# facebookresearch/co-tracker

Hardware: NVIDIA H100
Metric: tracked points*frames/sec at N=6400, T=16, 512^2 (higher is better)
Workload: dtype transformer + corr_mlp.fc2 + input_transform: bf16x3; correlation einsum: fp16x2; corr_mlp.fc1: bf16x3; fp32 accumulate, fp32 softmax/LayerNorm/GELU

## Files before the change

### cotracker_b200/csrc/common.cuh

```cuda
#pragma once
#include <cuda.h>
#include <cuda_bf16.h>
#include <cuda_fp16.h>
#include <cuda_runtime.h>
#include <stdint.h>

#include <atomic>

namespace ct3 {

struct DeviceOnce { std::atomic<uint64_t> done[2] = {}; };
template <typename F>
inline cudaError_t once_per_device(DeviceOnce& flag, F&& f) {
  int dev = 0;
  cudaError_t e = cudaGetDevice(&dev);
  if (e != cudaSuccess) return e;
  if (dev < 0 || dev >= 128) return f();
  const uint64_t bit = 1ull << (dev & 63);
  if (flag.done[dev >> 6].load(std::memory_order_acquire) & bit) return cudaSuccess;
  e = f();
  if (e == cudaSuccess) flag.done[dev >> 6].fetch_or(bit, std::memory_order_release);
  return e;
}

// ... 178 lines not shown
  uint64_t p;
  asm volatile("createpolicy.fractional.L2::evict_last.b64 %0, 1.0;" : "=l"(p));
  return p;
}
__device__ __forceinline__ void tma_load_4d_hint(void* smem_dst, const CUtensorMap* m, int c0, int c1, int c2, int c3,
                                                 uint64_t* bar, uint64_t policy) {
  asm volatile(
      "cp.async.bulk.tensor.4d.shared::cluster.global.mbarrier::complete_tx::bytes.L2::cache_hint [%0], [%1, {%3, %4, %5, %6}], [%2], %7;"
      ::"r"(smem_u32(smem_dst)), "l"(reinterpret_cast<uint64_t>(m)), "r"(smem_u32(bar)), "r"(c0), "r"(c1), "r"(c2),
      "r"(c3), "l"(policy)
      : "memory");
}
__device__ __forceinline__ void tma_load_3d(void* smem_dst, const CUtensorMap* m, int c0, int c1, int c2, uint64_t* bar) {
  asm volatile(
      "cp.async.bulk.tensor.3d.shared::cluster.global.mbarrier::complete_tx::bytes [%0], [%1, {%3, %4, %5}], [%2];"
      ::"r"(smem_u32(smem_dst)), "l"(reinterpret_cast<uint64_t>(m)), "r"(smem_u32(bar)), "r"(c0), "r"(c1), "r"(c2)
      : "memory");
}
__device__ __forceinline__ void tma_store_3d(const CUtensorMap* m, int c0, int c1, int c2, const void* smem_src) {
  asm volatile("cp.async.bulk.tensor.3d.global.shared::cta.bulk_group [%0, {%2, %3, %4}], [%1];"
               ::"l"(reinterpret_cast<uint64_t>(m)), "r"(smem_u32(smem_src)), "r"(c0), "r"(c1), "r"(c2)
               : "memory");
}

__device__ __forceinline__ void bulk_store_s2g(void* gdst, const void* ssrc, uint32_t bytes) {
  asm volatile("cp.async.bulk.global.shared::cta.bulk_group [%0], [%1], %2;" ::"l"(gdst), "r"(smem_u32(ssrc)), "r"(bytes)
               : "memory");
}
__device__ __forceinline__ void bulk_store_s2g_hint(void* gdst, const void* ssrc, uint32_t bytes, uint64_t policy) {
  asm volatile("cp.async.bulk.global.shared::cta.bulk_group.L2::cache_hint [%0], [%1], %2, %3;" ::"l"(gdst),
               "r"(smem_u32(ssrc)), "r"(bytes), "l"(policy)
               : "memory");
}
__device__ __forceinline__ void bulk_commit() { asm volatile("cp.async.bulk.commit_group;" ::: "memory"); }
__device__ __forceinline__ void bulk_wait_read0() { asm volatile("cp.async.bulk.wait_group.read 0;" ::: "memory"); }
__device__ __forceinline__ void bulk_wait0() { asm volatile("cp.async.bulk.wait_group 0;" ::: "memory"); }

__device__ __forceinline__ uint64_t gmma_desc_sw128(uint32_t smem_addr) {
  uint64_t d = 0;
  d |= (uint64_t)((smem_addr & 0x3FFFFu) >> 4);
  d |= (uint64_t)1 << 16;
  d |= (uint64_t)(1024 >> 4) << 32;
  d |= (uint64_t)1 << 62;
  return d;
}
__device__ __forceinline__ void wgmma_fence() { asm volatile("wgmma.fence.sync.aligned;" ::: "memory"); }
__device__ __forceinline__ void wgmma_commit() { asm volatile("wgmma.commit_group.sync.aligned;" ::: "memory"); }
template <int R>
__device__ __forceinline__ void wgmma_wait0(float (&d)[R]) {
  asm volatile("wgmma.wait_group.sync.aligned 0;" ::: "memory");
#pragma unroll
  for (int i = 0; i < R; ++i) asm volatile("" : "+f"(d[i])::"memory");
}

__device__ __forceinline__ void wgmma_m64n64_bf16(float (&d)[32], uint64_t da, uint64_t db, uint32_t scale_d) {
  asm volatile(
      "{\n\t.reg .pred p;\n\tsetp.ne.b32 p, %34, 0;\n\t"
      "wgmma.mma_async.sync.aligned.m64n64k16.f32.bf16.bf16 "
      "{%0, %1, %2, %3, %4, %5, %6, %7, %8, %9, %10, %11, %12, %13, %14, %15, %16, %17, %18, %19, %20, %21, %22, %23, %24, %25, %26, %27, %28, %29, %30, %31}, %32, %33, p, 1, 1, 0, 0;\n\t}"
      : "+f"(d[0]), "+f"(d[1]), "+f"(d[2]), "+f"(d[3]), "+f"(d[4]), "+f"(d[5]), "+f"(d[6]), "+f"(d[7]), "+f"(d[8]), "+f"(d[9]), "+f"(d[10]), "+f"(d[11]), "+f"(d[12]), "+f"(d[13]), "+f"(d[14]), "+f"(d[15]), "+f"(d[16]), "+f"(d[17]), "+f"(d[18]), "+f"(d[19]), "+f"(d[20]), "+f"(d[21]), "+f"(d[22]), "+f"(d[23]), "+f"(d[24]), "+f"(d[25]), "+f"(d[26]), "+f"(d[27]), "+f"(d[28]), "+f"(d[29]), "+f"(d[30]), "+f"(d[31])
      : "l"(da), "l"(db), "r"(scale_d));
}
__device__ __forceinline__ void wgmma_m64n128_bf16(float (&d)[64], uint64_t da, uint64_t db, uint32_t scale_d) {
  asm volatile(
      "{\n\t.reg .pred p;\n\tsetp.ne.b32 p, %66, 0;\n\t"
      "wgmma.mma_async.sync.aligned.m64n128k16.f32.bf16.bf16 "
      "{%0, %1, %2, %3, %4, %5, %6, %7, %8, %9, %10, %11, %12, %13, %14, %15, %16, %17, %18, %19, %20, %21, %22, %23, %24, %25, %26, %27, %28, %29, %30, %31, %32, %33, %34, %35, %36, %37, %38, %39, %40, %41, %42, %43, %44, %45, %46, %47, %48, %49, %50, %51, %52, %53, %54, %55, %56, %57, %58, %59, %60, %61, %62, %63}, %64, %65, p, 1, 1, 0, 0;\n\t}"
      : "+f"(d[0]), "+f"(d[1]), "+f"(d[2]), "+f"(d[3]), "+f"(d[4]), "+f"(d[5]), "+f"(d[6]), "+f"(d[7]), "+f"(d[8]), "+f"(d[9]), "+f"(d[10]), "+f"(d[11]), "+f"(d[12]), "+f"(d[13]), "+f"(d[14]), "+f"(d[15]), "+f"(d[16]), "+f"(d[17]), "+f"(d[18]), "+f"(d[19]), "+f"(d[20]), "+f"(d[21]), "+f"(d[22]), "+f"(d[23]), "+f"(d[24]), "+f"(d[25]), "+f"(d[26]), "+f"(d[27]), "+f"(d[28]), "+f"(d[29]), "+f"(d[30]), "+f"(d[31]), "+f"(d[32]), "+f"(d[33]), "+f"(d[34]), "+f"(d[35]), "+f"(d[36]), "+f"(d[37]), "+f"(d[38]), "+f"(d[39]), "+f"(d[40]), "+f"(d[41]), "+f"(d[42]), "+f"(d[43]), "+f"(d[44]), "+f"(d[45]), "+f"(d[46]), "+f"(d[47]), "+f"(d[48]), "+f"(d[49]), "+f"(d[50]), "+f"(d[51]), "+f"(d[52]), "+f"(d[53]), "+f"(d[54]), "+f"(d[55]), "+f"(d[56]), "+f"(d[57]), "+f"(d[58]), "+f"(d[59]), "+f"(d[60]), "+f"(d[61]), "+f"(d[62]), "+f"(d[63])
      : "l"(da), "l"(db), "r"(scale_d));
}
__device__ __forceinline__ void wgmma_m64n144_bf16(float (&d)[72], uint64_t da, uint64_t db, uint32_t scale_d) {
  asm volatile(
      "{\n\t.reg .pred p;\n\tsetp.ne.b32 p, %74, 0;\n\t"
      "wgmma.mma_async.sync.aligned.m64n144k16.f32.bf16.bf16 "
      "{%0, %1, %2, %3, %4, %5, %6, %7, %8, %9, %10, %11, %12, %13, %14, %15, %16, %17, %18, %19, %20, %21, %22, %23, %24, %25, %26, %27, %28, %29, %30, %31, %32, %33, %34, %35, %36, %37, %38, %39, %40, %41, %42, %43, %44, %45, %46, %47, %48, %49, %50, %51, %52, %53, %54, %55, %56, %57, %58, %59, %60, %61, %62, %63, %64, %65, %66, %67, %68, %69, %70, %71}, %72, %73, p, 1, 1, 0, 0;\n\t}"
      : "+f"(d[0]), "+f"(d[1]), "+f"(d[2]), "+f"(d[3]), "+f"(d[4]), "+f"(d[5]), "+f"(d[6]), "+f"(d[7]), "+f"(d[8]), "+f"(d[9]), "+f"(d[10]), "+f"(d[11]), "+f"(d[12]), "+f"(d[13]), "+f"(d[14]), "+f"(d[15]), "+f"(d[16]), "+f"(d[17]), "+f"(d[18]), "+f"(d[19]), "+f"(d[20]), "+f"(d[21]), "+f"(d[22]), "+f"(d[23]), "+f"(d[24]), "+f"(d[25]), "+f"(d[26]), "+f"(d[27]), "+f"(d[28]), "+f"(d[29]), "+f"(d[30]), "+f"(d[31]), "+f"(d[32]), "+f"(d[33]), "+f"(d[34]), "+f"(d[35]), "+f"(d[36]), "+f"(d[37]), "+f"(d[38]), "+f"(d[39]), "+f"(d[40]), "+f"(d[41]), "+f"(d[42]), "+f"(d[43]), "+f"(d[44]), "+f"(d[45]), "+f"(d[46]), "+f"(d[47]), "+f"(d[48]), "+f"(d[49]), "+f"(d[50]), "+f"(d[51]), "+f"(d[52]), "+f"(d[53]), "+f"(d[54]), "+f"(d[55]), "+f"(d[56]), "+f"(d[57]), "+f"(d[58]), "+f"(d[59]), "+f"(d[60]), "+f"(d[61]), "+f"(d[62]), "+f"(d[63]), "+f"(d[64]), "+f"(d[65]), "+f"(d[66]), "+f"(d[67]), "+f"(d[68]), "+f"(d[69]), "+f"(d[70]), "+f"(d[71])
      : "l"(da), "l"(db), "r"(scale_d));
}
__device__ __forceinline__ void wgmma_m64n64_f16(float (&d)[32], uint64_t da, uint64_t db, uint32_t scale_d) {
  asm volatile(
      "{\n\t.reg .pred p;\n\tsetp.ne.b32 p, %34, 0;\n\t"
      "wgmma.mma_async.sync.aligned.m64n64k16.f32.f16.f16 "
      "{%0, %1, %2, %3, %4, %5, %6, %7, %8, %9, %10, %11, %12, %13, %14, %15, %16, %17, %18, %19, %20, %21, %22, %23, %24, %25, %26, %27, %28, %29, %30, %31}, %32, %33, p, 1, 1, 0, 0;\n\t}"
      : "+f"(d[0]), "+f"(d[1]), "+f"(d[2]), "+f"(d[3]), "+f"(d[4]), "+f"(d[5]), "+f"(d[6]), "+f"(d[7]), "+f"(d[8]), "+f"(d[9]), "+f"(d[10]), "+f"(d[11]), "+f"(d[12]), "+f"(d[13]), "+f"(d[14]), "+f"(d[15]), "+f"(d[16]), "+f"(d[17]), "+f"(d[18]), "+f"(d[19]), "+f"(d[20]), "+f"(d[21]), "+f"(d[22]), "+f"(d[23]), "+f"(d[24]), "+f"(d[25]), "+f"(d[26]), "+f"(d[27]), "+f"(d[28]), "+f"(d[29]), "+f"(d[30]), "+f"(d[31])
      : "l"(da), "l"(db), "r"(scale_d));
}
__device__ __forceinline__ void wgmma_m64n128_f16(float (&d)[64], uint64_t da, uint64_t db, uint32_t scale_d) {
  asm volatile(
      "{\n\t.reg .pred p;\n\tsetp.ne.b32 p, %66, 0;\n\t"
      "wgmma.mma_async.sync.aligned.m64n128k16.f32.f16.f16 "
      "{%0, %1, %2, %3, %4, %5, %6, %7, %8, %9, %10, %11, %12, %13, %14, %15, %16, %17, %18, %19, %20, %21, %22, %23, %24, %25, %26, %27, %28, %29, %30, %31, %32, %33, %34, %35, %36, %37, %38, %39, %40, %41, %42, %43, %44, %45, %46, %47, %48, %49, %50, %51, %52, %53, %54, %55, %56, %57, %58, %59, %60, %61, %62, %63}, %64, %65, p, 1, 1, 0, 0;\n\t}"
      : "+f"(d[0]), "+f"(d[1]), "+f"(d[2]), "+f"(d[3]), "+f"(d[4]), "+f"(d[5]), "+f"(d[6]), "+f"(d[7]), "+f"(d[8]), "+f"(d[9]), "+f"(d[10]), "+f"(d[11]), "+f"(d[12]), "+f"(d[13]), "+f"(d[14]), "+f"(d[15]), "+f"(d[16]), "+f"(d[17]), "+f"(d[18]), "+f"(d[19]), "+f"(d[20]), "+f"(d[21]), "+f"(d[22]), "+f"(d[23]), "+f"(d[24]), "+f"(d[25]), "+f"(d[26]), "+f"(d[27]), "+f"(d[28]), "+f"(d[29]), "+f"(d[30]), "+f"(d[31]), "+f"(d[32]), "+f"(d[33]), "+f"(d[34]), "+f"(d[35]), "+f"(d[36]), "+f"(d[37]), "+f"(d[38]), "+f"(d[39]), "+f"(d[40]), "+f"(d[41]), "+f"(d[42]), "+f"(d[43]), "+f"(d[44]), "+f"(d[45]), "+f"(d[46]), "+f"(d[47]), "+f"(d[48]), "+f"(d[49]), "+f"(d[50]), "+f"(d[51]), "+f"(d[52]), "+f"(d[53]), "+f"(d[54]), "+f"(d[55]), "+f"(d[56]), "+f"(d[57]), "+f"(d[58]), "+f"(d[59]), "+f"(d[60]), "+f"(d[61]), "+f"(d[62]), "+f"(d[63])
      : "l"(da), "l"(db), "r"(scale_d));
}
__device__ __forceinline__ void wgmma_m64n144_f16(float (&d)[72], uint64_t da, uint64_t db, uint32_t scale_d) {
  asm volatile(
      "{\n\t.reg .pred p;\n\tsetp.ne.b32 p, %74, 0;\n\t"
      "wgmma.mma_async.sync.aligned.m64n144k16.f32.f16.f16 "
      "{%0, %1, %2, %3, %4, %5, %6, %7, %8, %9, %10, %11, %12, %13, %14, %15, %16, %17, %18, %19, %20, %21, %22, %23, %24, %25, %26, %27, %28, %29, %30, %31, %32, %33, %34, %35, %36, %37, %38, %39, %40, %41, %42, %43, %44, %45, %46, %47, %48, %49, %50, %51, %52, %53, %54, %55, %56, %57, %58, %59, %60, %61, %62, %63, %64, %65, %66, %67, %68, %69, %70, %71}, %72, %73, p, 1, 1, 0, 0;\n\t}"
      : "+f"(d[0]), "+f"(d[1]), "+f"(d[2]), "+f"(d[3]), "+f"(d[4]), "+f"(d[5]), "+f"(d[6]), "+f"(d[7]), "+f"(d[8]), "+f"(d[9]), "+f"(d[10]), "+f"(d[11]), "+f"(d[12]), "+f"(d[13]), "+f"(d[14]), "+f"(d[15]), "+f"(d[16]), "+f"(d[17]), "+f"(d[18]), "+f"(d[19]), "+f"(d[20]), "+f"(d[21]), "+f"(d[22]), "+f"(d[23]), "+f"(d[24]), "+f"(d[25]), "+f"(d[26]), "+f"(d[27]), "+f"(d[28]), "+f"(d[29]), "+f"(d[30]), "+f"(d[31]), "+f"(d[32]), "+f"(d[33]), "+f"(d[34]), "+f"(d[35]), "+f"(d[36]), "+f"(d[37]), "+f"(d[38]), "+f"(d[39]), "+f"(d[40]), "+f"(d[41]), "+f"(d[42]), "+f"(d[43]), "+f"(d[44]), "+f"(d[45]), "+f"(d[46]), "+f"(d[47]), "+f"(d[48]), "+f"(d[49]), "+f"(d[50]), "+f"(d[51]), "+f"(d[52]), "+f"(d[53]), "+f"(d[54]), "+f"(d[55]), "+f"(d[56]), "+f"(d[57]), "+f"(d[58]), "+f"(d[59]), "+f"(d[60]), "+f"(d[61]), "+f"(d[62]), "+f"(d[63]), "+f"(d[64]), "+f"(d[65]), "+f"(d[66]), "+f"(d[67]), "+f"(d[68]), "+f"(d[69]), "+f"(d[70]), "+f"(d[71])
      : "l"(da), "l"(db), "r"(scale_d));
}

__device__ __forceinline__ void wgmma_m64n48_bf16(float (&d)[24], uint64_t da, uint64_t db, uint32_t scale_d) {
  asm volatile(
      "{\n\t.reg .pred p;\n\tsetp.ne.b32 p, %26, 0;\n\t"
// ... 91 lines not shown
```

### cotracker_b200/csrc/gemm.cu

```cuda
#include "gemm.cuh"

namespace ct3 {
namespace {

constexpr int BM = 128, BN = 128, BK = 64;
constexpr int TILE_A = BM * BK * 2;
constexpr int TILE_B = BN * BK * 2;
constexpr int MMA_WARPS = 4;
constexpr int TMA_WARP = 4;
constexpr int EPI_WARP0 = 8;
constexpr int EPI_WARPS = 8;
constexpr int CW = 16;
constexpr int STG_WORDS = 32 * CW;
constexpr int MAX_STAGES = 4;
template <int NPROD>
struct Cfg {
  static constexpr int AP = NPROD >= 3 ? 2 : 1;
  static constexpr int BP = NPROD >= 2 ? 2 : 1;
  static constexpr int STAGE_BYTES = AP * TILE_A + BP * TILE_B;
  static constexpr int STAGES = NPROD >= 2 ? 2 : 4;
  static constexpr int OFF_B = AP * TILE_A;
};
constexpr int RING_BYTES = 2 * 65536;
static_assert(Cfg<1>::STAGES * Cfg<1>::STAGE_BYTES <= RING_BYTES && Cfg<2>::STAGES * Cfg<2>::STAGE_BYTES <= RING_BYTES &&
              Cfg<3>::STAGES * Cfg<3>::STAGE_BYTES <= RING_BYTES, "ring size");
constexpr int ACC_LD = BN + 4;
constexpr int OFF_ACC = RING_BYTES;
constexpr int OFF_STG = OFF_ACC + BM * ACC_LD * 4;
constexpr int OFF_BAR = OFF_STG + EPI_WARPS * STG_WORDS * 4;
constexpr int SMEM_BYTES = OFF_BAR + 256  + 1024 ;
static_assert(SMEM_BYTES <= 232448, "shared memory budget");
constexpr int THREADS = (EPI_WARP0 + EPI_WARPS) * 32;
constexpr int REG_TMA = 40, REG_MMA = 216, REG_EPI = 65536 / THREADS;
static_assert(128 * (REG_TMA + REG_MMA + 2 * REG_EPI) <= 65536, "register budget");

__device__ __forceinline__ float apply_act(float x, int act) {
  if (act == 1) return gelu_erf(x);
  if (act == 2) return gelu_tanh(x);
  return x;
}

__device__ __forceinline__ int stg_idx(int row, int word) { return row * CW + ((word + (row >> 1)) & (CW - 1)); }

__device__ __forceinline__ void epilogue_chunk(const GemmEpilogue& e, int M, int N, int row0, int col0, int lane,
                                               float (&v)[CW], uint32_t* stg) {
  const int row = row0 + lane;
  if (e.bias) {
    const float4* b4 = reinterpret_cast<const float4*>(e.bias + col0);
#pragma unroll
    for (int i = 0; i < CW / 4; ++i) {
      float4 b = __ldg(b4 + i);
      v[4 * i + 0] += b.x; v[4 * i + 1] += b.y; v[4 * i + 2] += b.z; v[4 * i + 3] += b.w;
    }
  }
  if (e.row_bias && row < M) {
    const float4* b4 = reinterpret_cast<const float4*>(e.row_bias + (int64_t)(row % e.row_mod) * N + col0);
#pragma unroll
    for (int i = 0; i < CW / 4; ++i) {
      float4 b = __ldg(b4 + i);
      v[4 * i + 0] += b.x; v[4 * i + 1] += b.y; v[4 * i + 2] += b.z; v[4 * i + 3] += b.w;
    }
  }
  if (e.act != 0) {
#pragma unroll
    for (int i = 0; i < CW; ++i) v[i] = apply_act(v[i], e.act);
  }
  const int rsub = lane >> 2, q = lane & 3;
  if (e.out_f32) {
#pragma unroll
    for (int c = 0; c < CW; ++c) stg[stg_idx(lane, c)] = __float_as_uint(v[c]);
    __syncwarp();
    float* base = e.out_f32 + (int64_t)(row0 + rsub) * e.ld_f32 + col0 + 4 * q;
    const int64_t rstep = 8 * e.ld_f32;
    float4 x[4];
#pragma unroll
    for (int k = 0; k < 4; ++k) {
      const int r = 8 * k + rsub;
      x[k] = make_float4(__uint_as_float(stg[stg_idx(r, 4 * q + 0)]), __uint_as_float(stg[stg_idx(r, 4 * q + 1)]),
                         __uint_as_float(stg[stg_idx(r, 4 * q + 2)]), __uint_as_float(stg[stg_idx(r, 4 * q + 3)]));
    }
    if (e.residual) {
      float4 r4[4];
#pragma unroll
      for (int k = 0; k < 4; ++k)
        r4[k] = (row0 + 8 * k + rsub < M) ? *reinterpret_cast<const float4*>(base + k * rstep) : make_float4(0.f, 0.f, 0.f, 0.f);
#pragma unroll
      for (int k = 0; k < 4; ++k) { x[k].x += r4[k].x; x[k].y += r4[k].y; x[k].z += r4[k].z; x[k].w += r4[k].w; }
    }
#pragma unroll
    for (int k = 0; k < 4; ++k)
      if (row0 + 8 * k + rsub < M) *reinterpret_cast<float4*>(base + k * rstep) = x[k];
    __syncwarp();
  }
  if (e.out_split) {
#pragma unroll
    for (int i = 0; i < CW / 2; ++i) {
      uint32_t hi, lo;
      split2(v[2 * i], v[2 * i + 1], hi, lo);
      stg[stg_idx(lane, i)] = hi;
      stg[stg_idx(lane, CW / 2 + i)] = lo;
    }
    __syncwarp();
    uint32_t off16_lane = 0xffffffffu;
    if (row < M) {
      const int orow = row / e.row_group;
      off16_lane = (uint32_t)(((long long)orow * e.ld_split + (long long)(row % e.row_group) * N + col0) >> 3);
    }
    uint4* plane = reinterpret_cast<uint4*>(e.out_split + (q >= 2 ? e.lo_off : 0)) + (q & 1);
#pragma unroll
    for (int k = 0; k < 4; ++k) {
      const int r = 8 * k + rsub;
      const uint32_t o16 = __shfl_sync(0xffffffffu, off16_lane, r);
      const uint4 w4 = make_uint4(stg[stg_idx(r, 4 * q + 0)], stg[stg_idx(r, 4 * q + 1)], stg[stg_idx(r, 4 * q + 2)],
                                  stg[stg_idx(r, 4 * q + 3)]);
      if (o16 != 0xffffffffu) plane[o16] = w4;
    }
    __syncwarp();
  }
}

template <int NPROD>
__global__ void __launch_bounds__(THREADS, 1)
gemm_split3_tc_kernel(const __grid_constant__ CUtensorMap tmX, const __grid_constant__ CUtensorMap tmW, int M,
                      int N, int Kpad, int fp16, GemmEpilogue epi) {
  using C = Cfg<NPROD>;
  constexpr int STAGES = C::STAGES, STAGE_BYTES = C::STAGE_BYTES;
  extern __shared__ __align__(1024) uint8_t smem_raw[];
  uint8_t* smem = smem_align1024(smem_raw);
  uint64_t* full_bar = reinterpret_cast<uint64_t*>(smem + OFF_BAR);
  uint64_t* empty_bar = full_bar + MAX_STAGES;
  uint64_t* tfull_bar = empty_bar + MAX_STAGES;
  uint64_t* tempty_bar = tfull_bar + 1;
  float* acc_tile = reinterpret_cast<float*>(smem + OFF_ACC);

  const int warp = threadIdx.x >> 5, lane = threadIdx.x & 31;

  if (threadIdx.x == 0) {
    tma_prefetch_desc(&tmX);
    tma_prefetch_desc(&tmW);
    for (int i = 0; i < STAGES; ++i) {
      mbar_init(&full_bar[i], 1);
      mbar_init(&empty_bar[i], MMA_WARPS);
    }
    mbar_init(tfull_bar, MMA_WARPS);
    mbar_init(tempty_bar, EPI_WARPS * 32);
    fence_barrier_init();
  }
  __syncthreads();

  const int num_mt = (M + BM - 1) / BM;
  const int num_nt = N / BN;
  const int num_tiles = num_mt * num_nt;
  const int num_kb = Kpad / BK;

  if (warp >= MMA_WARPS && warp < EPI_WARP0) {
    setmaxnreg_dec<REG_TMA>();
    if (warp == TMA_WARP && elect_one()) {
      int stage = 0;
      uint32_t phase = 0;
      for (int tile = blockIdx.x; tile < num_tiles; tile += gridDim.x) {
        const int mt = tile / num_nt, nt = tile % num_nt;
        for (int kb = 0; kb < num_kb; ++kb) {
          mbar_wait(&empty_bar[stage], phase ^ 1u);
          mbar_arrive_expect_tx(&full_bar[stage], STAGE_BYTES);
          uint8_t* s = smem + stage * STAGE_BYTES;
          tma_load_2d(s, &tmX, kb * BK, mt * BM, &full_bar[stage]);
          if (C::AP == 2) tma_load_2d(s + TILE_A, &tmX, Kpad + kb * BK, mt * BM, &full_bar[stage]);
          tma_load_2d(s + C::OFF_B, &tmW, kb * BK, nt * BN, &full_bar[stage]);
          if (C::BP == 2) tma_load_2d(s + C::OFF_B + TILE_B, &tmW, Kpad + kb * BK, nt * BN, &full_bar[stage]);
          if (++stage == STAGES) { stage = 0; phase ^= 1u; }
        }
      }
    }
  } else if (warp < MMA_WARPS) {
    setmaxnreg_inc<REG_MMA>();
    int stage = 0;
    uint32_t phase = 0, acc_phase = 0;
    for (int tile = blockIdx.x; tile < num_tiles; tile += gridDim.x) {
      float d0[BN / 2], d1[BN / 2];
      for (int kb = 0; kb < num_kb; ++kb) {
        mbar_wait(&full_bar[stage], phase);
        wgmma_fence();
        const uint32_t sa = smem_u32(smem + stage * STAGE_BYTES);
        if (fp16) mma_kblock<NPROD, BN, true>(d0, d1, sa, TILE_A, C::OFF_B, TILE_B, kb == 0);
        else mma_kblock<NPROD, BN, false>(d0, d1, sa, TILE_A, C::OFF_B, TILE_B, kb == 0);
        wgmma_commit();
        wgmma_wait0(d0);
        wgmma_wait0(d1);
        __syncwarp();
        if (lane == 0) mbar_arrive(&empty_bar[stage]);
        if (++stage == STAGES) { stage = 0; phase ^= 1u; }
      }
      mbar_wait(tempty_bar, acc_phase ^ 1u);
      acc_store<BN>(d0, acc_tile, ACC_LD);
      acc_store<BN>(d1, acc_tile + 64 * ACC_LD, ACC_LD);
      __syncwarp();
      if (lane == 0) mbar_arrive(tfull_bar);
      acc_phase ^= 1u;
    }
  } else {
    const int e = warp - EPI_WARP0;
    const int quarter = e & 3;
    constexpr int CH = BN / CW / (EPI_WARPS / 4);
    const int chunk0 = (e >> 2) * CH;
    uint32_t acc_phase = 0;
    for (int tile = blockIdx.x; tile < num_tiles; tile += gridDim.x) {
      const int mt = tile / num_nt, nt = tile % num_nt;
      mbar_wait(tfull_bar, acc_phase);
      const int row0 = mt * BM + quarter * 32;
      uint32_t* stg = reinterpret_cast<uint32_t*>(smem + OFF_STG) + e * STG_WORDS;
      const float* arow = acc_tile + (quarter * 32 + lane) * ACC_LD;
#pragma unroll 1
      for (int chunk = chunk0; chunk < chunk0 + CH; ++chunk) {
        float v[CW];
        acc_row_ld<CW>(arow + chunk * CW, v);
        epilogue_chunk(epi, M, N, row0, nt * BN + chunk * CW, lane, v, stg);
      }
      mbar_arrive(tempty_bar);
      acc_phase ^= 1u;
    }
  }
}

namespace qa {
constexpr int BNQ = 144;
constexpr int TILE_BQ = BNQ * BK * 2;
constexpr int STAGE = 2 * TILE_A + 2 * TILE_BQ;
constexpr int NSTAGE = 2;
constexpr int QACC_LD = BNQ + 4;
constexpr int QOFF_ACC = NSTAGE * STAGE;
constexpr int OFF_BARQ = QOFF_ACC + BM * QACC_LD * 4;
constexpr int SMEM = OFF_BARQ + 256 + 1024;
constexpr int EPIW = 4;
constexpr int QEPI_WARP0 = 8;
constexpr int NTHREADS = 12 * 32;
constexpr int REG_PRODUCER = 40, REG_COMPUTE = 232;
static_assert(128 * (REG_PRODUCER + 2 * REG_COMPUTE) <= NTHREADS * 168, "register budget");
static_assert(SMEM <= 232448, "shared memory budget");
}

__global__ void __launch_bounds__(qa::NTHREADS, 1)
gemm_qkv_time_attn_kernel(const __grid_constant__ CUtensorMap tmX, const __grid_constant__ CUtensorMap tmW, int M,
                          int Kpad, int T, int R, float scale_log2e, GemmEpilogue epi) {
  using namespace qa;
  extern __shared__ __align__(1024) uint8_t smem_raw[];
  uint8_t* smem = smem_align1024(smem_raw);
  uint64_t* full_bar = reinterpret_cast<uint64_t*>(smem + OFF_BARQ);
  uint64_t* empty_bar = full_bar + NSTAGE;
  uint64_t* tfull_bar = empty_bar + NSTAGE;
  uint64_t* tempty_bar = tfull_bar + 1;
  float* acc = reinterpret_cast<float*>(smem + QOFF_ACC);

  const int warp = threadIdx.x >> 5, lane = threadIdx.x & 31;
  if (threadIdx.x == 0) {
    tma_prefetch_desc(&tmX);
    tma_prefetch_desc(&tmW);
    for (int i = 0; i < NSTAGE; ++i) {
      mbar_init(&full_bar[i], 1);
      mbar_init(&empty_bar[i], MMA_WARPS);
    }
    mbar_init(tfull_bar, MMA_WARPS);
    mbar_init(tempty_bar, EPIW * 32);
    fence_barrier_init();
  }
  __syncthreads();

  const int num_mt = (M + R - 1) / R;
  const int num_tiles = num_mt * kHeads;
  const int num_kb = Kpad / BK;

  if (warp >= MMA_WARPS && warp < QEPI_WARP0) {
    setmaxnreg_dec<REG_PRODUCER>();
    if (warp == TMA_WARP && elect_one()) {
      int stage = 0;
      uint32_t phase = 0;
      for (int tile = blockIdx.x; tile < num_tiles; tile += gridDim.x) {
        const int mt = tile / kHeads, h = tile % kHeads;
        for (int kb = 0; kb < num_kb; ++kb) {
          mbar_wait(&empty_bar[stage], phase ^ 1u);
          mbar_arrive_expect_tx(&full_bar[stage], STAGE);
          uint8_t* s = smem + stage * STAGE;
          tma_load_2d(s, &tmX, kb * BK, mt * R, &full_bar[stage]);
          tma_load_2d(s + TILE_A, &tmX, Kpad + kb * BK, mt * R, &full_bar[stage]);
          tma_load_2d(s + 2 * TILE_A, &tmW, kb * BK, h * BNQ, &full_bar[stage]);
          tma_load_2d(s + 2 * TILE_A + TILE_BQ, &tmW, Kpad + kb * BK, h * BNQ, &full_bar[stage]);
          if (++stage == NSTAGE) { stage = 0; phase ^= 1u; }
        }
      }
    }
  } else if (warp < MMA_WARPS) {
    setmaxnreg_inc<REG_COMPUTE>();
    int stage = 0;
    uint32_t phase = 0, acc_phase = 0;
    for (int tile = blockIdx.x; tile < num_tiles; tile += gridDim.x) {
      float d0[BNQ / 2], d1[BNQ / 2];
      for (int kb = 0; kb < num_kb; ++kb) {
        mbar_wait(&full_bar[stage], phase);
        wgmma_fence();
        mma_kblock<3, BNQ, false>(d0, d1, smem_u32(smem + stage * STAGE), TILE_A, 2 * TILE_A, TILE_BQ, kb == 0);
        wgmma_commit();
        wgmma_wait0(d0);
        wgmma_wait0(d1);
        __syncwarp();
        if (lane == 0) mbar_arrive(&empty_bar[stage]);
        if (++stage == NSTAGE) { stage = 0; phase ^= 1u; }
      }
      mbar_wait(tempty_bar, acc_phase ^ 1u);
      acc_store<BNQ>(d0, acc, QACC_LD);
      acc_store<BNQ>(d1, acc + 64 * QACC_LD, QACC_LD);
      __syncwarp();
      if (lane == 0) mbar_arrive(tfull_bar);
      acc_phase ^= 1u;
    }
  } else {
    setmaxnreg_inc<REG_COMPUTE>();
    const int r = (warp - QEPI_WARP0) * 32 + lane;
    const int tracks = R / T;
    const int jtrack = min(r / T, tracks - 1);
    const float* kbase = acc + (int64_t)jtrack * T * QACC_LD + kDh;
    float* arow = acc + r * QACC_LD;
    uint32_t acc_phase = 0;
    for (int tile = blockIdx.x; tile < num_tiles; tile += gridDim.x) {
      const int mt = tile / kHeads, h = tile % kHeads;
      mbar_wait(tfull_bar, acc_phase);
      acc_phase ^= 1u;
      float xq[kDh];
// ... 146 lines not shown
  }
  for (int i = 0; i < 4; ++i)
    for (int j = 0; j < 4; ++j) {
      const int r = m0 + ty * 4 + i, c = n0 + tx * 4 + j;
      if (r < M && c < N) epilogue_store1(epi, N, r, c, acc[i][j]);
    }
}

typedef CUresult (*EncodeTiledFn)(CUtensorMap*, CUtensorMapDataType, cuuint32_t, void*, const cuuint64_t*,
                                  const cuuint64_t*, const cuuint32_t*, const cuuint32_t*, CUtensorMapInterleave,
                                  CUtensorMapSwizzle, CUtensorMapL2promotion, CUtensorMapFloatOOBfill);

EncodeTiledFn get_encode_fn() {
  static const EncodeTiledFn fn = [] {
    void* p = nullptr;
    cudaDriverEntryPointQueryResult q;
    if (cudaGetDriverEntryPoint("cuTensorMapEncodeTiled", &p, cudaEnableDefault, &q) == cudaSuccess &&
        q == cudaDriverEntryPointSuccess)
      return reinterpret_cast<EncodeTiledFn>(p);
    return (EncodeTiledFn) nullptr;
  }();
  return fn;
}

bool make_tmap(CUtensorMap* m, const void* base, uint64_t rows, uint64_t cols, uint32_t box_rows = 128) {
  EncodeTiledFn fn = get_encode_fn();
  if (!fn) return false;
  cuuint64_t dims[2] = {cols, rows};
  cuuint64_t strides[1] = {cols * 2};
  cuuint32_t box[2] = {64, box_rows};
  cuuint32_t estr[2] = {1, 1};
  CUresult r = fn(m, CU_TENSOR_MAP_DATA_TYPE_BFLOAT16, 2, const_cast<void*>(base), dims, strides, box, estr,
                  CU_TENSOR_MAP_INTERLEAVE_NONE, CU_TENSOR_MAP_SWIZZLE_128B, CU_TENSOR_MAP_L2_PROMOTION_L2_128B,
                  CU_TENSOR_MAP_FLOAT_OOB_FILL_NONE);
  return r == CUDA_SUCCESS;
}

}

bool encode_tensor_map(CUtensorMap* m, CUtensorMapDataType dtype, int rank, const void* base, const uint64_t* dims,
                       const uint64_t* strides_bytes, const uint32_t* box, CUtensorMapSwizzle swizzle) {
  EncodeTiledFn fn = get_encode_fn();
  if (!fn || rank < 1 || rank > 5) return false;
  cuuint64_t d[5], st[5];
  cuuint32_t b[5], es[5];
  for (int i = 0; i < rank; ++i) { d[i] = dims[i]; b[i] = box[i]; es[i] = 1; }
  for (int i = 0; i + 1 < rank; ++i) st[i] = strides_bytes[i];
  return fn(m, dtype, (cuuint32_t)rank, const_cast<void*>(base), d, st, b, es, CU_TENSOR_MAP_INTERLEAVE_NONE, swizzle,
            CU_TENSOR_MAP_L2_PROMOTION_L2_256B, CU_TENSOR_MAP_FLOAT_OOB_FILL_NONE) == CUDA_SUCCESS;
}

namespace {

template <int NPROD>
cudaError_t launch_tc(const GemmProblem& p, const CUtensorMap& tmX, const CUtensorMap& tmW, int num_mt, int num_sms,
                      cudaStream_t stream) {
  static DeviceOnce attr;
  cudaError_t e = once_per_device(attr, [&] {
    return cudaFuncSetAttribute(gemm_split3_tc_kernel<NPROD>, cudaFuncAttributeMaxDynamicSharedMemorySize, SMEM_BYTES);
  });
  if (e != cudaSuccess) return e;
  const int num_tiles = num_mt * (p.N / BN);
  const int grid = num_tiles < num_sms ? num_tiles : num_sms;
  gemm_split3_tc_kernel<NPROD><<<grid, THREADS, SMEM_BYTES, stream>>>(tmX, tmW, p.M, p.N, p.Kpad, p.fp16, p.epi);
  return cudaGetLastError();
}

}

bool qkv_time_attn_supported(int T) { return T >= 1 && T <= BM; }

int gemm_qkv_time_attn_launch(const __nv_bfloat16* x_split, const __nv_bfloat16* w_heads, const float* bias_heads,
                              int M, int Kpad, int T, __nv_bfloat16* att_split, int64_t ld_split, int lo_off,
                              float scale, int num_sms, cudaStream_t stream, const char** err) {
  *err = nullptr;
  if (M <= 0 || Kpad <= 0 || (Kpad % BK) != 0 || !qkv_time_attn_supported(T) || (M % T) != 0) {
    *err = "qkv_time_attn: need M > 0, M % T == 0, 1 <= T <= 128, Kpad % 64 == 0";
    return (int)cudaErrorInvalidValue;
  }
  if (((reinterpret_cast<uintptr_t>(x_split) | reinterpret_cast<uintptr_t>(w_heads) |
        reinterpret_cast<uintptr_t>(att_split)) & 15) || (ld_split % 8) != 0 || (lo_off % 8) != 0) {
    *err = "qkv_time_attn: operands must be 16-byte aligned";
    return (int)cudaErrorInvalidValue;
  }
  const int R = (BM / T) * T;
  CUtensorMap tmX, tmW;
  if (!make_tmap(&tmX, x_split, (uint64_t)M, 2ull * Kpad) ||
      !make_tmap(&tmW, w_heads, (uint64_t)(kHeads * qa::BNQ), 2ull * Kpad, (uint32_t)qa::BNQ)) {
    *err = "qkv_time_attn: cuTensorMapEncodeTiled failed";
    return (int)cudaErrorInvalidValue;
  }
  static DeviceOnce attr;
  cudaError_t e = once_per_device(attr, [&] {
    return cudaFuncSetAttribute(gemm_qkv_time_attn_kernel, cudaFuncAttributeMaxDynamicSharedMemorySize, qa::SMEM);
  });
  if (e != cudaSuccess) { *err = "qkv_time_attn: cudaFuncSetAttribute failed"; return (int)e; }
  const int num_tiles = ((M + R - 1) / R) * kHeads;
  GemmEpilogue epi;
  epi.bias = bias_heads;
  epi.out_split = att_split;
  epi.ld_split = ld_split;
  epi.lo_off = lo_off;
  gemm_qkv_time_attn_kernel<<<num_tiles < num_sms ? num_tiles : num_sms, qa::NTHREADS, qa::SMEM, stream>>>(
      tmX, tmW, M, Kpad, T, R, scale * 1.44269504088896340736f, epi);
  return (int)cudaGetLastError();
}

const char* gemm_check(const GemmProblem& p) {
  if (p.M <= 0 || p.N <= 0 || p.Kpad <= 0 || (p.N % BN) != 0 || (p.Kpad % BK) != 0)
    return "gemm: need M>0, N % 128 == 0, Kpad % 64 == 0";
  if (p.products < 1 || p.products > 3 || p.fp16 < 0 || p.fp16 > 1) return "gemm: products in 1..3, fp16 in 0..1";
  const int64_t x_ld = p.x_ld ? p.x_ld : 2 * (int64_t)p.Kpad;
  if (x_ld < (p.products == 3 ? 2 : 1) * (int64_t)p.Kpad || (x_ld % 8) != 0)
    return "gemm: x_ld too small for the operand planes this product count reads";
  if ((reinterpret_cast<uintptr_t>(p.x_split) | reinterpret_cast<uintptr_t>(p.w_split)) & 15)
    return "gemm: operands must be 16-byte aligned";
  const GemmEpilogue& e = p.epi;
  if (!e.out_f32 && !e.out_split) return "gemm: no output";
// ... 38 lines not shown
```

Before: 649,600.

## Use ping-pong consumer warpgroups with register epilogue for long-K split GEMMs

For GEMMs with K above 384, the old layout (one MMA warpgroup, a TMA warp and separate epilogue warps fed through an smem accumulator tile) is replaced by two consumer warpgroups that alternate tiles. Each group signals the other when its mainloop is done, then runs the epilogue straight from registers via small per-warp staging buffers. The ring grows to 192KB with more stages, the wgmma wait keeps one group in flight, and fp16 becomes a template parameter. Short-K GEMMs keep the old kernel. This aims to overlap epilogue with MMA and drop the accumulator round-trip through smem, at the cost of more registers per consumer and more complex barrier phase logic.

```diff
diff --git a/cotracker_b200/csrc/common.cuh b/cotracker_b200/csrc/common.cuh
--- a/cotracker_b200/csrc/common.cuh
+++ b/cotracker_b200/csrc/common.cuh
@@ -254,6 +254,7 @@
 #pragma unroll
   for (int i = 0; i < R; ++i) asm volatile("" : "+f"(d[i])::"memory");
 }
+__device__ __forceinline__ void wgmma_wait1() { asm volatile("wgmma.wait_group.sync.aligned 1;" ::: "memory"); }
 
 __device__ __forceinline__ void wgmma_m64n64_bf16(float (&d)[32], uint64_t da, uint64_t db, uint32_t scale_d) {
   asm volatile(
diff --git a/cotracker_b200/csrc/gemm.cu b/cotracker_b200/csrc/gemm.cu
--- a/cotracker_b200/csrc/gemm.cu
+++ b/cotracker_b200/csrc/gemm.cu
@@ -7,32 +7,30 @@
 constexpr int TILE_A = BM * BK * 2;
 constexpr int TILE_B = BN * BK * 2;
 constexpr int MMA_WARPS = 4;
-constexpr int TMA_WARP = 4;
-constexpr int EPI_WARP0 = 8;
+constexpr int CONSUMER_WARP0 = 4;
 constexpr int EPI_WARPS = 8;
 constexpr int CW = 16;
 constexpr int STG_WORDS = 32 * CW;
-constexpr int MAX_STAGES = 4;
+constexpr int FRAG_LD = CW + 4;
+constexpr int FRAG_STG_WORDS = 32 * FRAG_LD;
+constexpr int MAX_STAGES = 6;
+constexpr int RING_BYTES = 3 * 65536;
 template <int NPROD>
 struct Cfg {
   static constexpr int AP = NPROD >= 3 ? 2 : 1;
   static constexpr int BP = NPROD >= 2 ? 2 : 1;
   static constexpr int STAGE_BYTES = AP * TILE_A + BP * TILE_B;
-  static constexpr int STAGES = NPROD >= 2 ? 2 : 4;
+  static constexpr int STAGES = RING_BYTES / STAGE_BYTES;
   static constexpr int OFF_B = AP * TILE_A;
+  static_assert(STAGES >= 3 && STAGES <= MAX_STAGES && STAGES * STAGE_BYTES == RING_BYTES, "ring");
 };
-constexpr int RING_BYTES = 2 * 65536;
-static_assert(Cfg<1>::STAGES * Cfg<1>::STAGE_BYTES <= RING_BYTES && Cfg<2>::STAGES * Cfg<2>::STAGE_BYTES <= RING_BYTES &&
-              Cfg<3>::STAGES * Cfg<3>::STAGE_BYTES <= RING_BYTES, "ring size");
-constexpr int ACC_LD = BN + 4;
-constexpr int OFF_ACC = RING_BYTES;
-constexpr int OFF_STG = OFF_ACC + BM * ACC_LD * 4;
-constexpr int OFF_BAR = OFF_STG + EPI_WARPS * STG_WORDS * 4;
+constexpr int OFF_STG = RING_BYTES;
+constexpr int OFF_BAR = OFF_STG + EPI_WARPS * FRAG_STG_WORDS * 4;
 constexpr int SMEM_BYTES = OFF_BAR + 256  + 1024 ;
 static_assert(SMEM_BYTES <= 232448, "shared memory budget");
-constexpr int THREADS = (EPI_WARP0 + EPI_WARPS) * 32;
-constexpr int REG_TMA = 40, REG_MMA = 216, REG_EPI = 65536 / THREADS;
-static_assert(128 * (REG_TMA + REG_MMA + 2 * REG_EPI) <= 65536, "register budget");
+constexpr int THREADS = 3 * 128;
+constexpr int REG_TMA = 40, REG_MMA = 232;
+static_assert(128 * (REG_TMA + 2 * REG_MMA) <= 65536, "register budget");
 
 __device__ __forceinline__ float apply_act(float x, int act) {
   if (act == 1) return gelu_erf(x);
@@ -119,19 +117,134 @@
   }
 }
 
-template <int NPROD>
+__device__ __forceinline__ int stg_row(int row0, int r) { return row0 + r + ((r & 16) ? 48 : 0); }
+
+__device__ __forceinline__ void epilogue_frag(const GemmEpilogue& e, int M, int N, int row0, int col0, int lane,
+                                              float (&f)[4][4], uint32_t* stg) {
+  const int fr = lane >> 2, fc = 2 * (lane & 3);
+  if (e.bias) {
+#pragma unroll
+    for (int jj = 0; jj < 2; ++jj) {
+      const float2 b = __ldg(reinterpret_cast<const float2*>(e.bias + col0 + 8 * jj + fc));
+#pragma unroll
+      for (int m = 0; m < 4; ++m) { f[m][2 * jj] += b.x; f[m][2 * jj + 1] += b.y; }
+    }
+  }
+  if (e.row_bias) {
+#pragma unroll
+    for (int m = 0; m < 4; ++m) {
+      const int r = stg_row(row0, fr + 8 * m);
+      if (r < M) {
+        const float* rb = e.row_bias + (int64_t)(r % e.row_mod) * N + col0 + fc;
+#pragma unroll
+        for (int jj = 0; jj < 2; ++jj) {
+          const float2 b = __ldg(reinterpret_cast<const float2*>(rb + 8 * jj));
+          f[m][2 * jj] += b.x; f[m][2 * jj + 1] += b.y;
+        }
+      }
+    }
+  }
+  if (e.act != 0) {
+#pragma unroll
+    for (int m = 0; m < 4; ++m)
+#pragma unroll
+      for (int i = 0; i < 4; ++i) f[m][i] = apply_act(f[m][i], e.act);
+  }
+  const int rsub = lane >> 2, q = lane & 3;
+  const uint4* sq = reinterpret_cast<const uint4*>(stg + rsub * FRAG_LD) + q;
+  float* xw = reinterpret_cast<float*>(stg) + fr * FRAG_LD + fc;
+  if (e.out_f32) {
+#pragma unroll
+    for (int m = 0; m < 4; ++m)
+#pragma unroll
+      for (int jj = 0; jj < 2; ++jj)
+        *reinterpret_cast<float2*>(xw + 8 * m * FRAG_LD + 8 * jj) = make_float2(f[m][2 * jj], f[m][2 * jj + 1]);
+    __syncwarp();
+    float* base = e.out_f32 + (int64_t)(row0 + rsub) * e.ld_f32 + col0 + 4 * q;
+    float4 x[4];
+#pragma unroll
+    for (int k = 0; k < 4; ++k) {
+      const uint4 w4 = sq[k * 8 * FRAG_LD / 4];
+      x[k] = make_float4(__uint_as_float(w4.x), __uint_as_float(w4.y), __uint_as_float(w4.z), __uint_as_float(w4.w));
+    }
+    if (e.residual) {
+      float4 r4[4];
+#pragma unroll
+      for (int k = 0; k < 4; ++k)
+        r4[k] = (stg_row(row0, 8 * k + rsub) < M) ? *reinterpret_cast<const float4*>(base + stg_row(0, 8 * k) * e.ld_f32)
+                                                   : make_float4(0.f, 0.f, 0.f, 0.f);
+#pragma unroll
+      for (int k = 0; k < 4; ++k) { x[k].x += r4[k].x; x[k].y += r4[k].y; x[k].z += r4[k].z; x[k].w += r4[k].w; }
+    }
+#pragma unroll
+    for (int k = 0; k < 4; ++k)
+      if (stg_row(row0, 8 * k + rsub) < M) *reinterpret_cast<float4*>(base + stg_row(0, 8 * k) * e.ld_f32) = x[k];
+    __syncwarp();
+  }
+  if (e.out_split) {
+    uint32_t* xs = stg + fr * FRAG_LD + (lane & 3);
+#pragma unroll
+    for (int m = 0; m < 4; ++m)
+#pragma unroll
+      for (int jj = 0; jj < 2; ++jj) {
+        uint32_t hi, lo;
+        split2(f[m][2 * jj], f[m][2 * jj + 1], hi, lo);
+        xs[8 * m * FRAG_LD + 4 * jj] = hi;
+        xs[8 * m * FRAG_LD + CW / 2 + 4 * jj] = lo;
+      }
+    __syncwarp();
+    const int row = stg_row(row0, lane);
+    uint32_t off16_lane = 0xffffffffu;
+    if (row < M) {
+      const int orow = row / e.row_group;
+      off16_lane = (uint32_t)(((long long)orow * e.ld_split + (long long)(row % e.row_group) * N + col0) >> 3);
+    }
+    uint4* plane = reinterpret_cast<uint4*>(e.out_split + (q >= 2 ? e.lo_off : 0)) + (q & 1);
+#pragma unroll
+    for (int k = 0; k < 4; ++k) {
+      const uint32_t o16 = __shfl_sync(0xffffffffu, off16_lane, 8 * k + rsub);
+      const uint4 w4 = sq[k * 8 * FRAG_LD / 4];
+      if (o16 != 0xffffffffu) plane[o16] = w4;
+    }
+    __syncwarp();
+  }
+}
+
+template <int NPROD, bool F16>
+__device__ __forceinline__ void mma_tile(float (&d0)[BN / 2], float (&d1)[BN / 2], uint8_t* smem, uint64_t* full_bar,
+                                         uint64_t* empty_bar, uint64_t* turn_other, uint32_t g, int num_kb, int lane) {
+  using C = Cfg<NPROD>;
+  for (int kb = 0; kb < num_kb; ++kb, ++g) {
+    const uint32_t slot = g % C::STAGES;
+    mbar_wait(&full_bar[slot], (g / C::STAGES) & 1u);
+    wgmma_fence();
+    mma_kblock<NPROD, BN, F16>(d0, d1, smem_u32(smem + slot * C::STAGE_BYTES), TILE_A, C::OFF_B, TILE_B, kb == 0);
+    wgmma_commit();
+    if (kb > 0) {
+      wgmma_wait1();
+      __syncwarp();
+      if (lane == 0) mbar_arrive(&empty_bar[(g - 1) % C::STAGES]);
+    }
+  }
+  __syncwarp();
+  if (lane == 0) mbar_arrive(turn_other);
+  wgmma_wait0(d0);
+  wgmma_wait0(d1);
+  __syncwarp();
+  if (lane == 0) mbar_arrive(&empty_bar[(g - 1) % C::STAGES]);
+}
+
+template <int NPROD, bool F16>
 __global__ void __launch_bounds__(THREADS, 1)
 gemm_split3_tc_kernel(const __grid_constant__ CUtensorMap tmX, const __grid_constant__ CUtensorMap tmW, int M,
-                      int N, int Kpad, int fp16, GemmEpilogue epi) {
+                      int N, int Kpad, GemmEpilogue epi) {
   using C = Cfg<NPROD>;
   constexpr int STAGES = C::STAGES, STAGE_BYTES = C::STAGE_BYTES;
   extern __shared__ __align__(1024) uint8_t smem_raw[];
   uint8_t* smem = smem_align1024(smem_raw);
   uint64_t* full_bar = reinterpret_cast<uint64_t*>(smem + OFF_BAR);
   uint64_t* empty_bar = full_bar + MAX_STAGES;
-  uint64_t* tfull_bar = empty_bar + MAX_STAGES;
-  uint64_t* tempty_bar = tfull_bar + 1;
-  float* acc_tile = reinterpret_cast<float*>(smem + OFF_ACC);
+  uint64_t* turn_bar = empty_bar + MAX_STAGES;
 
   const int warp = threadIdx.x >> 5, lane = threadIdx.x & 31;
 
@@ -142,20 +255,18 @@
       mbar_init(&full_bar[i], 1);
       mbar_init(&empty_bar[i], MMA_WARPS);
     }
-    mbar_init(tfull_bar, MMA_WARPS);
-    mbar_init(tempty_bar, EPI_WARPS * 32);
+    mbar_init(&turn_bar[0], MMA_WARPS);
+    mbar_init(&turn_bar[1], MMA_WARPS);
     fence_barrier_init();
   }
   __syncthreads();
 
-  const int num_mt = (M + BM - 1) / BM;
   const int num_nt = N / BN;
-  const int num_tiles = num_mt * num_nt;
+  const int num_tiles = ((M + BM - 1) / BM) * num_nt;
   const int num_kb = Kpad / BK;
-
-  if (warp >= MMA_WARPS && warp < EPI_WARP0) {
+  if (warp < CONSUMER_WARP0) {
     setmaxnreg_dec<REG_TMA>();
-    if (warp == TMA_WARP && elect_one()) {
+    if (warp == 0 && elect_one()) {
       int stage = 0;
       uint32_t phase = 0;
       for (int tile = blockIdx.x; tile < num_tiles; tile += gridDim.x) {
@@ -172,8 +283,108 @@
         }
       }
     }
+  } else {
+    setmaxnreg_inc<REG_MMA>();
+    const int c = warp / 4 - 1, w = warp & 3;
+    uint32_t* stg = reinterpret_cast<uint32_t*>(smem + OFF_STG) + (warp - CONSUMER_WARP0) * FRAG_STG_WORDS;
+    for (int pos = c, tile = blockIdx.x + c * gridDim.x; tile < num_tiles; pos += 2, tile += 2 * gridDim.x) {
+      if (pos > 0) mbar_wait(&turn_bar[c], (uint32_t)((pos - 1) >> 1) & 1u);
+      float d0[BN / 2], d1[BN / 2];
+      const uint32_t g = (uint32_t)pos * (uint32_t)num_kb;
+      mma_tile<NPROD, F16>(d0, d1, smem, full_bar, empty_bar, &turn_bar[c ^ 1], g, num_kb, lane);
+
+      const int mt = tile / num_nt, nt = tile % num_nt;
+      const int row0 = mt * BM + 16 * w;
+#pragma unroll
+      for (int ch = 0; ch < BN / CW; ++ch) {
+        float f[4][4];
+#pragma unroll
+        for (int jj = 0; jj < 2; ++jj) {
+          const int j = 2 * ch + jj;
+          f[0][2 * jj] = d0[4 * j]; f[0][2 * jj + 1] = d0[4 * j + 1];
+          f[1][2 * jj] = d0[4 * j + 2]; f[1][2 * jj + 1] = d0[4 * j + 3];
+          f[2][2 * jj] = d1[4 * j]; f[2][2 * jj + 1] = d1[4 * j + 1];
+          f[3][2 * jj] = d1[4 * j + 2]; f[3][2 * jj + 1] = d1[4 * j + 3];
+        }
+        epilogue_frag(epi, M, N, row0, nt * BN + ch * CW, lane, f, stg);
+      }
+    }
+  }
+}
+
+constexpr int SHORT_K = 384;
+namespace hk {
+constexpr int RING = 2 * 65536;
+template <int NPROD>
+struct Ring { static constexpr int STAGES = NPROD >= 2 ? 2 : 4; };
+constexpr int ACC_LD = BN + 4;
+constexpr int OFF_ACC = RING;
+constexpr int OFF_STG = OFF_ACC + BM * ACC_LD * 4;
+constexpr int OFF_BAR = OFF_STG + EPI_WARPS * STG_WORDS * 4;
+constexpr int SMEM = OFF_BAR + 256 + 1024;
+static_assert(SMEM <= 232448, "shared memory budget");
+constexpr int TMA_WARP = 4, EPI_WARP0 = 8;
+constexpr int NTHREADS = (EPI_WARP0 + EPI_WARPS) * 32;
+constexpr int REG_TMA = 40, REG_MMA = 216, REG_EPI = 65536 / NTHREADS;
+static_assert(128 * (REG_TMA + REG_MMA + 2 * REG_EPI) <= 65536, "register budget");
+static_assert(Ring<1>::STAGES * Cfg<1>::STAGE_BYTES <= RING && Ring<3>::STAGES * Cfg<3>::STAGE_BYTES <= RING, "ring size");
+}
+
+template <int NPROD>
+__global__ void __launch_bounds__(hk::NTHREADS, 1)
+gemm_split3_tc_short_k_kernel(const __grid_constant__ CUtensorMap tmX, const __grid_constant__ CUtensorMap tmW, int M,
+                              int N, int Kpad, int fp16, GemmEpilogue epi) {
+  constexpr int STAGES = hk::Ring<NPROD>::STAGES, STAGE_BYTES = Cfg<NPROD>::STAGE_BYTES;
+  using C = Cfg<NPROD>;
+  extern __shared__ __align__(1024) uint8_t smem_raw[];
+  uint8_t* smem = smem_align1024(smem_raw);
+  uint64_t* full_bar = reinterpret_cast<uint64_t*>(smem + hk::OFF_BAR);
+  uint64_t* empty_bar = full_bar + MAX_STAGES;
+  uint64_t* tfull_bar = empty_bar + MAX_STAGES;
+  uint64_t* tempty_bar = tfull_bar + 1;
+  float* acc_tile = reinterpret_cast<float*>(smem + hk::OFF_ACC);
+
+  const int warp = threadIdx.x >> 5, lane = threadIdx.x & 31;
+
+  if (threadIdx.x == 0) {
+    tma_prefetch_desc(&tmX);
+    tma_prefetch_desc(&tmW);
+    for (int i = 0; i < STAGES; ++i) {
+      mbar_init(&full_bar[i], 1);
+      mbar_init(&empty_bar[i], MMA_WARPS);
+    }
+    mbar_init(tfull_bar, MMA_WARPS);
+    mbar_init(tempty_bar, EPI_WARPS * 32);
+    fence_barrier_init();
+  }
+  __syncthreads();
+
+  const int num_mt = (M + BM - 1) / BM;
+  const int num_nt = N / BN;
+  const int num_tiles = num_mt * num_nt;
+  const int num_kb = Kpad / BK;
+
+  if (warp >= MMA_WARPS && warp < hk::EPI_WARP0) {
+    setmaxnreg_dec<hk::REG_TMA>();
+    if (warp == hk::TMA_WARP && elect_one()) {
+      int stage = 0;
+      uint32_t phase = 0;
+      for (int tile = blockIdx.x; tile < num_tiles; tile += gridDim.x) {
+        const int mt = tile / num_nt, nt = tile % num_nt;
+        for (int kb = 0; kb < num_kb; ++kb) {
+          mbar_wait(&empty_bar[stage], phase ^ 1u);
+          mbar_arrive_expect_tx(&full_bar[stage], STAGE_BYTES);
+          uint8_t* s = smem + stage * STAGE_BYTES;
+          tma_load_2d(s, &tmX, kb * BK, mt * BM, &full_bar[stage]);
+          if (C::AP == 2) tma_load_2d(s + TILE_A, &tmX, Kpad + kb * BK, mt * BM, &full_bar[stage]);
+          tma_load_2d(s + C::OFF_B, &tmW, kb * BK, nt * BN, &full_bar[stage]);
+          if (C::BP == 2) tma_load_2d(s + C::OFF_B + TILE_B, &tmW, Kpad + kb * BK, nt * BN, &full_bar[stage]);
+          if (++stage == STAGES) { stage = 0; phase ^= 1u; }
+        }
+      }
+    }
   } else if (warp < MMA_WARPS) {
-    setmaxnreg_inc<REG_MMA>();
+    setmaxnreg_inc<hk::REG_MMA>();
     int stage = 0;
     uint32_t phase = 0, acc_phase = 0;
     for (int tile = blockIdx.x; tile < num_tiles; tile += gridDim.x) {
@@ -192,14 +403,14 @@
         if (++stage == STAGES) { stage = 0; phase ^= 1u; }
       }
       mbar_wait(tempty_bar, acc_phase ^ 1u);
-      acc_store<BN>(d0, acc_tile, ACC_LD);
-      acc_store<BN>(d1, acc_tile + 64 * ACC_LD, ACC_LD);
+      acc_store<BN>(d0, acc_tile, hk::ACC_LD);
+      acc_store<BN>(d1, acc_tile + 64 * hk::ACC_LD, hk::ACC_LD);
       __syncwarp();
       if (lane == 0) mbar_arrive(tfull_bar);
       acc_phase ^= 1u;
     }
   } else {
-    const int e = warp - EPI_WARP0;
+    const int e = warp - hk::EPI_WARP0;
     const int quarter = e & 3;
     constexpr int CH = BN / CW / (EPI_WARPS / 4);
     const int chunk0 = (e >> 2) * CH;
@@ -208,8 +419,8 @@
       const int mt = tile / num_nt, nt = tile % num_nt;
       mbar_wait(tfull_bar, acc_phase);
       const int row0 = mt * BM + quarter * 32;
-      uint32_t* stg = reinterpret_cast<uint32_t*>(smem + OFF_STG) + e * STG_WORDS;
-      const float* arow = acc_tile + (quarter * 32 + lane) * ACC_LD;
+      uint32_t* stg = reinterpret_cast<uint32_t*>(smem + hk::OFF_STG) + e * STG_WORDS;
+      const float* arow = acc_tile + (quarter * 32 + lane) * hk::ACC_LD;
 #pragma unroll 1
       for (int chunk = chunk0; chunk < chunk0 + CH; ++chunk) {
         float v[CW];
@@ -232,6 +443,7 @@
 constexpr int OFF_BARQ = QOFF_ACC + BM * QACC_LD * 4;
 constexpr int SMEM = OFF_BARQ + 256 + 1024;
 constexpr int EPIW = 4;
+constexpr int QTMA_WARP = 4;
 constexpr int QEPI_WARP0 = 8;
 constexpr int NTHREADS = 12 * 32;
 constexpr int REG_PRODUCER = 40, REG_COMPUTE = 232;
@@ -271,7 +483,7 @@
 
   if (warp >= MMA_WARPS && warp < QEPI_WARP0) {
     setmaxnreg_dec<REG_PRODUCER>();
-    if (warp == TMA_WARP && elect_one()) {
+    if (warp == QTMA_WARP && elect_one()) {
       int stage = 0;
       uint32_t phase = 0;
       for (int tile = blockIdx.x; tile < num_tiles; tile += gridDim.x) {
@@ -524,18 +736,39 @@
 
 namespace {
 
-template <int NPROD>
+template <int NPROD, bool F16>
 cudaError_t launch_tc(const GemmProblem& p, const CUtensorMap& tmX, const CUtensorMap& tmW, int num_mt, int num_sms,
                       cudaStream_t stream) {
   static DeviceOnce attr;
   cudaError_t e = once_per_device(attr, [&] {
-    return cudaFuncSetAttribute(gemm_split3_tc_kernel<NPROD>, cudaFuncAttributeMaxDynamicSharedMemorySize, SMEM_BYTES);
+    return cudaFuncSetAttribute(gemm_split3_tc_kernel<NPROD, F16>, cudaFuncAttributeMaxDynamicSharedMemorySize,
+                                SMEM_BYTES);
   });
   if (e != cudaSuccess) return e;
   const int num_tiles = num_mt * (p.N / BN);
   const int grid = num_tiles < num_sms ? num_tiles : num_sms;
-  gemm_split3_tc_kernel<NPROD><<<grid, THREADS, SMEM_BYTES, stream>>>(tmX, tmW, p.M, p.N, p.Kpad, p.fp16, p.epi);
+  gemm_split3_tc_kernel<NPROD, F16><<<grid, THREADS, SMEM_BYTES, stream>>>(tmX, tmW, p.M, p.N, p.Kpad, p.epi);
   return cudaGetLastError();
+}
+
+template <int NPROD>
+cudaError_t launch_tc(const GemmProblem& p, const CUtensorMap& tmX, const CUtensorMap& tmW, int num_mt, int num_sms,
+                      cudaStream_t stream) {
+  const int num_tiles = num_mt * (p.N / BN);
+  const int grid = num_tiles < num_sms ? num_tiles : num_sms;
+  if (p.Kpad <= SHORT_K) {
+    static DeviceOnce attr;
+    cudaError_t e = once_per_device(attr, [&] {
+      return cudaFuncSetAttribute(gemm_split3_tc_short_k_kernel<NPROD>, cudaFuncAttributeMaxDynamicSharedMemorySize,
+                                  hk::SMEM);
+    });
+    if (e != cudaSuccess) return e;
+    gemm_split3_tc_short_k_kernel<NPROD><<<grid, hk::NTHREADS, hk::SMEM, stream>>>(tmX, tmW, p.M, p.N, p.Kpad, p.fp16,
+                                                                                 p.epi);
+    return cudaGetLastError();
+  }
+  return p.fp16 ? launch_tc<NPROD, true>(p, tmX, tmW, num_mt, num_sms, stream)
+                : launch_tc<NPROD, false>(p, tmX, tmW, num_mt, num_sms, stream);
 }
 
 }
```

After: 660,000 (median of 6 runs). +1.6%, better.
